# meg89/bevfusion_multimodal_3d_object_detection

Measured on AMD Instinct MI355X. Metric: BEV frames/sec (6-cam+LiDAR, 128x128 BEV), higher is better.
Workload: dtype fp32; 1 GPU; camera+LiDAR, 6x900x1600 images + 35k-point sweep, BEV 128x128; batch_per_gpu=8, parallelism=replicas x1, conv_kernels=wino, weights=random-init (synthetic, seeded), launch=eager, mode=inference forward -> 5 head tensors

## Files before the change

### bevfusion_multimodal_3d_object_detection_amd/_lib.py

```python
from __future__ import annotations

import ctypes as C
import os
from typing import Optional, Sequence

import torch

_HERE = os.path.dirname(os.path.abspath(__file__))
LIB_PATH = os.path.join(_HERE, "csrc", "libbevf_hip.so")


class BevfError(RuntimeError):
    pass


class ConvDesc(C.Structure):
    _fields_ = [("x", C.c_void_p), ("w", C.c_void_p), ("scale", C.c_void_p), ("shift", C.c_void_p),
                ("res", C.c_void_p), ("y", C.c_void_p), ("colmax", C.c_void_p)] + \
               [(n, C.c_int32) for n in ("N", "H", "W", "Cin", "x_cs", "Ho", "Wo", "Cout", "y_cs", "res_cs",
                                         "KH", "KW", "stride", "pad", "relu", "rows_per_group", "tile")] + \
               [(n, C.c_void_p) for n in ("stats", "stats_pivot", "bnb_x", "bnb_y", "bnb_mean", "bnb_invstd", "bnb_gamma",
                                          "bnb_beta")]


# ... 100 lines not shown
    "bevf_pillar_moments_f32": (C.c_int, [C.POINTER(PillarGeom)] + [C.c_void_p] * 4 + [C.c_int, C.c_float, C.c_float] +
                                [C.c_void_p] * 10),
    "bevf_pillar_pfn_backward_f32": (C.c_int, [C.POINTER(PillarGeom)] + [C.c_void_p] * 10 + [C.c_int] * 2 + [C.c_void_p] * 6),
    "bevf_resize_normalize_u8": (C.c_int, [C.c_void_p] * 2 + [C.c_int] * 5 + [C.c_void_p] * 2 + [C.c_int] + [C.c_void_p] * 2 +
                                 [C.c_int] + [C.POINTER(C.c_float)] * 2 + [C.c_void_p]),
    "bevf_lidar_filter_pad_f32": (C.c_int, [C.c_void_p] * 5 + [C.c_int] * 3 + [C.POINTER(C.c_float), C.c_void_p]),
    "bevf_resample_tables_box_f64": (C.c_int, [C.c_void_p] + [C.c_int] * 7 + [C.c_void_p] * 5),
    "bevf_resize_crop_u8": (C.c_int, [C.c_void_p] * 3 + [C.c_int] * 5 + [C.c_void_p] * 2 + [C.c_int] + [C.c_void_p] * 2 + [C.c_int] +
                            [C.c_void_p]),
    "bevf_jitter_flip_normalize_u8": (C.c_int, [C.c_void_p] * 5 + [C.c_int] * 3 + [C.POINTER(C.c_float)] * 2 + [C.c_void_p]),
    "bevf_points_affine_work_floats": (C.c_size_t, [C.c_int] * 3),
    "bevf_points_affine_filter_pad_f32": (C.c_int, [C.c_void_p] * 6 + [C.c_int] * 6 + [C.POINTER(C.c_float), C.c_void_p]),
    "bevf_points_affine_f32": (C.c_int, [C.c_void_p] * 3 + [C.c_float] + [C.c_int] * 5 + [C.c_void_p]),
    "bevf_boxes_affine_f32": (C.c_int, [C.c_void_p] * 5 + [C.c_int] * 3 + [C.c_void_p]),
    "bevf_split_weights_f32x3": (C.c_int, [C.c_void_p, C.c_void_p, C.c_size_t, C.c_void_p]),
    "bevf_conv2d_nhwc_f32x3": (C.c_int, [C.POINTER(ConvDesc), C.c_void_p]),
    "bevf_conv2d_nhwc_bf16": (C.c_int, [C.POINTER(ConvDesc), C.c_void_p]),
    "bevf_conv3x3_pack_elems": (C.c_size_t, [C.c_int] * 2),
    "bevf_conv3x3_bf16_ct": (C.c_int, [C.c_int]),
    "bevf_conv3x3_pack_bf16": (C.c_int, [C.c_void_p] * 2 + [C.c_int] * 2 + [C.c_void_p]),
    "bevf_conv3x3_bf16": (C.c_int, [C.POINTER(ConvDesc), C.c_void_p]),
    "bevf_debug_conv3x3_stamps": (C.c_int, [C.c_void_p]),
    "bevf_debug_wino_stamps": (C.c_int, [C.c_void_p]),
    "bevf_stem_pack_bf16": (C.c_int, [C.c_void_p] * 3),
    "bevf_stem_conv7x7_bf16mma": (C.c_int, [C.c_void_p] * 5 + [C.c_int] * 4 + [C.c_void_p]),
    "bevf_stem_pool_bf16mma": (C.c_int, [C.c_void_p] * 5 + [C.c_int] * 3 + [C.c_void_p]),
    "bevf_stem_conv7x7_bf16out": (C.c_int, [C.c_void_p] * 5 + [C.c_int] * 4 + [C.c_void_p]),
    "bevf_maxpool3x3s2_nhwc_bf16": (C.c_int, [C.c_void_p] * 2 + [C.c_int] * 4 + [C.c_void_p]),
    "bevf_pointwise_smallk_bf16out": (C.c_int, [C.c_void_p] * 5 + [C.c_int] * 4 + [C.c_void_p]),
    "bevf_linear_bf16w": (C.c_int, [C.c_void_p] * 4 + [C.c_int] * 7 + [C.c_void_p]),
    "bevf_cam_mean_bf16": (C.c_int, [C.c_void_p] * 2 + [C.c_int] * 4 + [C.c_void_p]),
    "bevf_bilinear_nhwc_bf16": (C.c_int, [C.c_void_p] * 2 + [C.c_int] * 8 + [C.c_void_p]),
    "bevf_broadcast_nhwc_bf16": (C.c_int, [C.c_void_p] * 2 + [C.c_int] * 4 + [C.c_void_p]),
    "bevf_expand_border_classes_bf16": (C.c_int, [C.c_void_p] * 2 + [C.c_int] * 5 + [C.c_void_p]),
    "bevf_head_tail_bf16": (C.c_int, [C.POINTER(HeadDesc), C.c_void_p]),
    "bevf_conv_pixtab_bytes": (C.c_size_t, [C.c_int] * 7),
    "bevf_conv_pixtab": (C.c_int, [C.c_void_p] + [C.c_int] * 8 + [C.c_void_p]),
    "bevf_conv2d_wgrad_f32": (C.c_int, [C.POINTER(WgradDesc), C.c_void_p]),
    "bevf_wino_wgrad_workspace_floats": (C.c_size_t, [C.c_int] * 5),
    "bevf_wino_wgrad_table_bytes": (C.c_size_t, [C.c_int] * 3),
    "bevf_wino_wgrad_table": (C.c_int, [C.c_void_p] + [C.c_int] * 5 + [C.c_void_p]),
    "bevf_conv3x3_wgrad_wino_f32": (C.c_int, [C.POINTER(WgradDesc), C.c_void_p, C.c_int, C.c_void_p]),
    "bevf_zero_stuff_nhwc_f32": (C.c_int, [C.c_void_p] * 2 + [C.c_int] * 7 + [C.c_void_p]),
    "bevf_stem_wgrad_f32": (C.c_int, [C.c_void_p] * 3 + [C.c_int] * 3 + [C.c_void_p]),
    "bevf_interleave2x2_nhwc_f32": (C.c_int, [C.c_void_p] * 4 + [C.c_int] * 4 + [C.c_void_p]),
    "bevf_bn_work_floats": (C.c_size_t, [C.c_int]),
# ... 1143 lines not shown
```

### bevfusion_multimodal_3d_object_detection_amd/csrc/conv_wino.hip

```cpp
#include "wino_common.h"

namespace {

struct WinoArgs {
  const float* x;
  const float* u;
  const float* scale;
  const float* shift;
  const float* res;
  float* y;
  float* stats;
  const float* pivot;
  const float *bnb_x, *bnb_y, *bnb_mean, *bnb_invstd, *bnb_gamma, *bnb_beta;
  int N, H, W, Cin, x_cs, Cout, y_cs, res_cs;
  int TBY, TBX, nct;
  int HS, SB;
  unsigned div_mul;
  unsigned long long* stamps;
};

constexpr int kWinoStamps = 6;

constexpr int PITCH = 36;
constexpr int PDMA = 12;
constexpr int PATCH_FLOATS = 4 * PDMA * 64 * 4;
constexpr int BG_FLOATS = 16 * 4 * 16 * 8;
constexpr int LDS_BYTES = (2 * PATCH_FLOATS + 2 * BG_FLOATS) * 4;

template <bool RES, bool RELU, bool STATS = false, int BNB = 0, int GEO = 0, bool DIAG = false>
__global__ __launch_bounds__(256, 1) void wino_f32(const WinoArgs p) {
  auto stamp_at = [&](int i, unsigned long long tm) {
    if constexpr (DIAG) {
      if (threadIdx.x == 0) p.stamps[(size_t)((blockIdx.z * gridDim.y + blockIdx.y) * gridDim.x + blockIdx.x) * kWinoStamps + i] = tm;
    }
  };
  auto stamp = [&](int i) {
    if constexpr (DIAG) stamp_at(i, __builtin_amdgcn_s_memtime());
  };
  stamp(0);
  constexpr int BHP = GEO ? 32 : 16, BWP = GEO ? 8 : 16;
  constexpr int PWP = BWP + 2, PIXG = (BHP + 2) * PWP;
  constexpr int PSLOTSG = PIXG * 9;
  static_assert(PSLOTSG <= 4 * PDMA * 64, "patch does not fit the DMA image");
  extern __shared__ __attribute__((aligned(16))) float lds[];
  float* const patch = lds;
  float* const bbuf = lds + 2 * PATCH_FLOATS;
  const int tid = threadIdx.x, lane = tid & 63;
  const int wave = __builtin_amdgcn_readfirstlane(tid >> 6);
  const int G = p.Cin >> 3;
  const int NCH = p.Cin >> 5;
  const __amdgpu_buffer_rsrc_t rsx = buf_rsrc(p.x);
  auto block_rows = [&](int sp, int& n0, int& r0, int& n, int& rb, int& hw) {
    if (p.HS) {
      const int s0 = BHP * sp - 1 + p.HS, q0 = (int)__umulhi((unsigned)s0, p.div_mul);
      n0 = q0 - 1;
      r0 = s0 - q0 * p.HS;
      hw = p.HS;
      const bool top = r0 + 1 == p.HS;
      n = top ? q0 : n0;
      rb = top ? 0 : r0 + 1;
    } else {
      n0 = p.div_mul ? (int)__umulhi((unsigned)sp, p.div_mul) : sp;
      rb = BHP * (sp - n0 * p.TBY);
      r0 = rb - 1;
      hw = 0x7fffffff;
      n = n0;
    }
  };
  auto wrap_row = [](int& row, int hw) {
    const bool wr = row >= hw;
    row -= wr ? hw : 0;
    return wr;
  };
  auto pixel_off = [&](unsigned pix, int n0, int r0, int hw, int ix0, bool& ok) {
    const unsigned py = __umul24(pix, GEO ? 6554u : 3641u) >> 16, px = pix - __umul24(py, (unsigned)PWP);
    int iy = r0 + (int)py;
    const int ix = ix0 + (int)px;
    const bool wr = wrap_row(iy, hw);
    ok = (unsigned)iy < (unsigned)p.H && (unsigned)ix < (unsigned)p.W && (unsigned)(n0 + (wr ? 1 : 0)) < (unsigned)p.N;
    const unsigned row = (unsigned)(n0 * p.H) + (wr ? (unsigned)p.H : 0u) + (unsigned)iy;
    return __umul24(__umul24(row, (unsigned)p.W) + (unsigned)ix, (unsigned)(p.x_cs * 4));
  };
  auto patch_dma_from = [&](__amdgpu_buffer_rsrc_t rs, unsigned voff, unsigned soff, int buf, int j) {
    __builtin_amdgcn_raw_ptr_buffer_load_lds(rs, (__attribute__((address_space(3))) void*)(patch + buf * PATCH_FLOATS + (4 * j + wave) * 256),
                                             16, voff, soff, 0, 0);
  };
  auto patch_dma = [&](unsigned voff, unsigned soff, int buf, int j) { patch_dma_from(rsx, voff, soff, buf, j); };
  auto make_pv = [&](unsigned (&pv)[PDMA], int& n, int& rb, int& hw, int& bx, int& ct) {
    bx = blockIdx.x;
    ct = blockIdx.z;
    int n0, r0;
    block_rows(blockIdx.y, n0, r0, n, rb, hw);
    const int ix0 = BWP * bx - 1;
#pragma unroll
    for (int j = 0; j < PDMA; ++j) {
      const unsigned sl = (unsigned)((4 * j + wave) * 64 + lane);
      const unsigned pix = __umul24(sl, 7282u) >> 16, piece = sl - 9u * pix;
      bool pok;
      const unsigned off = pixel_off(pix, n0, r0, hw, ix0, pok);
      const bool in_patch = (4 * j + 3) * 64 + 63 < PSLOTSG || sl < (unsigned)PSLOTSG;
      pv[j] = (in_patch && piece < 8u && pok) ? off + 16u * piece : kOob;
      patch_dma(pv[j], 0, 0, j);
      __builtin_amdgcn_sched_barrier(0);
    }
  };
  const __amdgpu_buffer_rsrc_t rsr_pf = buf_rsrc(RES ? p.res : p.x);
  bool pf_res = false;

  const __amdgpu_buffer_rsrc_t rsu = buf_rsrc(p.u);
  const unsigned u_lane = (unsigned)((wave * 8 * 256 + lane * 4) * 4);
  auto dma_piece = [&](unsigned img, int buf, int i) {
    __builtin_amdgcn_raw_ptr_buffer_load_lds(rsu, (__attribute__((address_space(3))) void*)(bbuf + buf * BG_FLOATS + wave * 8 * 256 + i * 256),
                                             16, u_lane, img + i * 1024, 0, 0);
  };

  const int t = lane & 15, kq = lane >> 4;
  const int ty = GEO ? 4 * wave + (t >> 2) : 2 * wave + (t >> 3), tx = GEO ? (t & 3) : (t & 7);
  const int a_lane = ((2 * ty) * PWP + 2 * tx) * PITCH + 2 * kq;
  const int b_lane = kq * 64 + t * 4;

  f32x4 acc[16][4];
  f32x2 vv[2][16], dn[16];
  auto load_patch = [&](const float* pa, int q, int c) {
    dn[4 * q + c] = *reinterpret_cast<const f32x2*>(pa + (q * PWP + c) * PITCH);
    dn[4 * q + c + 1] = *reinterpret_cast<const f32x2*>(pa + (q * PWP + c + 1) * PITCH);
  };
  auto transform_into = [&](f32x2 (&v)[16]) {
#pragma unroll
    for (int c = 0; c < 4; ++c) {
      const f32x2 t0 = dn[0 + c] - dn[8 + c], t1 = dn[4 + c] + dn[8 + c], t2 = dn[8 + c] - dn[4 + c], t3 = dn[4 + c] - dn[12 + c];
      dn[0 + c] = t0; dn[4 + c] = t1; dn[8 + c] = t2; dn[12 + c] = t3;
    }
#pragma unroll
    for (int r = 0; r < 4; ++r) {
      v[4 * r + 0] = dn[4 * r + 0] - dn[4 * r + 2];
      v[4 * r + 1] = dn[4 * r + 1] + dn[4 * r + 2];
      v[4 * r + 2] = dn[4 * r + 2] - dn[4 * r + 1];
      v[4 * r + 3] = dn[4 * r + 1] - dn[4 * r + 3];
    }
  };

  unsigned pv[PDMA], pvl[PDMA];
  int n, rb, hw, bx, ct;
  {
    const int ct0 = blockIdx.z;
#pragma unroll
    for (int i = 0; i < 8; ++i) dma_piece((unsigned)(ct0 * G) * (BG_FLOATS * 4), 0, i);
  }
  make_pv(pv, n, rb, hw, bx, ct);
  unsigned long long t_issued = 0;
  if constexpr (DIAG) t_issued = __builtin_amdgcn_s_memtime();
#pragma unroll
  for (int j = 0; j < 4; ++j) patch_dma(NCH > 1 ? pv[j] : kOob, 128, 1, j);
  asm volatile("s_waitcnt vmcnt(4) lgkmcnt(0)\n\ts_barrier" ::: "memory");
#pragma unroll
  for (int q = 0; q < 4; ++q) {
    load_patch(patch + a_lane, q, 0);
    load_patch(patch + a_lane, q, 2);
  }
  transform_into(vv[0]);
  int pbuf = 0;
  stamp_at(1, t_issued);
  stamp(2);

  auto group = [&](auto glc, auto firstc, const unsigned psoff, const unsigned bimg, const bool bnext) {
    constexpr int gl = decltype(glc)::value;
    constexpr bool kFirst = decltype(firstc)::value;
    const int abuf = gl == 3 ? pbuf ^ 1 : pbuf;
    constexpr int agl = (gl + 1) & 3;
    const float* pb = bbuf + (gl & 1) * BG_FLOATS + b_lane;
    const float* pa = patch + abuf * PATCH_FLOATS + a_lane + agl * 8;
    f32x4 b0[2], b1[2];
    b0[0] = *reinterpret_cast<const f32x4*>(pb);
    b0[1] = *reinterpret_cast<const f32x4*>(pb + 256);
#pragma unroll
    for (int f = 0; f < 16; ++f) {
      f32x4 (&bc)[2] = (f & 1) ? b1 : b0;
      f32x4 (&bn)[2] = (f & 1) ? b0 : b1;
      const f32x2 a = vv[gl & 1][f];
#pragma unroll
      for (int k = 0; k < 8; ++k) {
        const int j = k >> 2, nb = k & 3;
        if (kFirst && j == 0) MFMA0(acc[f][nb], a[j], bc[nb >> 1][(nb & 1) * 2 + j]);
        else MFMA(acc[f][nb], a[j], bc[nb >> 1][(nb & 1) * 2 + j]);
        if (k == 0 && f < 15) bn[0] = *reinterpret_cast<const f32x4*>(pb + ((f + 1) * 2) * 256);
        if (k == 1 && f < 15) bn[1] = *reinterpret_cast<const f32x4*>(pb + ((f + 1) * 2 + 1) * 256);
        if (f < 4) {
          if (k == 2) load_patch(pa, f, 0);
          if (k == 3) load_patch(pa, f, 2);
        }
        if (f == 5 && k == 2) transform_into(vv[(gl + 1) & 1]);
        if (f == 0 && bnext) dma_piece(bimg, (gl + 1) & 1, k);
        if (f == 1 && k >= 4 && gl != 2) {
          constexpr int part = gl == 3 ? 0 : gl + 1;
          if (RES && gl == 0 && pf_res) patch_dma_from(rsr_pf, pvl[part * 4 + (k - 4)], psoff, pbuf ^ 1, part * 4 + (k - 4));
          else patch_dma(pvl[part * 4 + (k - 4)], psoff, gl == 3 ? pbuf : pbuf ^ 1, part * 4 + (k - 4));
        }
        __builtin_amdgcn_sched_barrier(0);
      }
    }
    if constexpr (gl == 3) asm volatile("s_nop 15\n\ts_nop 15\n\ts_waitcnt vmcnt(4) lgkmcnt(0)\n\ts_barrier" ::: "memory");
    else asm volatile("s_waitcnt vmcnt(%0) lgkmcnt(0)\n\ts_barrier" ::"n"(gl == 2 ? 0 : 4) : "memory");
  };

  {
    using T = std::true_type;
    using F = std::false_type;
#pragma unroll
    for (int j = 0; j < PDMA; ++j) pvl[j] = pv[j];
    for (int chunk = 0; chunk < NCH; ++chunk) {
      const bool lastc = chunk + 1 == NCH;
      const unsigned ug = (unsigned)(ct * G + chunk * 4) * (BG_FLOATS * 4), gb = BG_FLOATS * 4;
      const unsigned soff = (unsigned)((chunk + 1) * 128);
      if (lastc) {
#pragma unroll
        for (int j = 4; j < PDMA; ++j) pvl[j] = kOob;
        if constexpr (RES) {
          pf_res = true;
#pragma unroll
          for (int s2 = 0; s2 < 2; ++s2) {
            const int line = s2 * 64 + lane, pw = line >> 1;
            const int prow = GEO ? (pw >> 3) : (pw >> 4), pcol = GEO ? (pw & 7) : (pw & 15);
            int ry = rb + (GEO ? 8 : 4) * wave + prow;
            const bool wr = wrap_row(ry, hw);
            const int rn = n + (wr ? 1 : 0), rx = BWP * bx + pcol;
            const bool ok = rn < p.N && ry < p.H && rx < p.W && ct * 64 + (line & 1) * 32 < p.Cout;
            pvl[4 + s2] = ok ? (unsigned)((((rn * p.H + ry) * p.W + rx) * p.res_cs + ct * 64 + (line & 1) * 32) * 4) - soff : kOob;
          }
        }
      }
      if (chunk + 2 >= NCH) {
#pragma unroll
        for (int j = 0; j < 4; ++j) pvl[j] = kOob;
      }
      if (chunk == 0) group(ic<0>{}, T{}, soff, ug + 1 * gb, true); else group(ic<0>{}, F{}, soff, ug + 1 * gb, true);
      group(ic<1>{}, F{}, soff, ug + 2 * gb, true);
      group(ic<2>{}, F{}, soff, ug + 3 * gb, true);
      group(ic<3>{}, F{}, soff + 128, ug + 4 * gb, !lastc);
      pbuf ^= 1;
    }

    asm volatile("s_waitcnt vmcnt(0)");
    stamp(3);
    if constexpr (STATS || BNB != 0) __syncthreads();
    {
      int oy = rb + (GEO ? 8 * wave + 2 * kq : 4 * wave + 2 * (kq >> 1));
      const int ox = GEO ? 8 * bx : 16 * bx + 8 * (kq & 1);
      const bool wr = wrap_row(oy, hw);
      const int nl = n + (wr ? 1 : 0);
      const bool rok[2] = {nl < p.N && oy < p.H, nl < p.N && oy + 1 < p.H};
      const bool interior = BWP * bx + BWP <= p.W && ct * 64 + 64 <= p.Cout;
      const __amdgpu_buffer_rsrc_t rsy = buf_rsrc(p.y);
      const __amdgpu_buffer_rsrc_t rsr = buf_rsrc(p.res);
      const unsigned y_lane = (unsigned)((((nl * p.H + oy) * p.W + ox) * p.y_cs + ct * 64 + t) * 4);
      const unsigned r_lane = (unsigned)((((nl * p.H + oy) * p.W + ox) * p.res_cs + ct * 64 + t) * 4);
      const unsigned yb[2] = {rok[0] ? y_lane : kOob, rok[1] ? y_lane + (unsigned)(p.W * p.y_cs * 4) : kOob};
      const unsigned rbs[2] = {rok[0] ? r_lane : kOob, rok[1] ? r_lane + (unsigned)(p.W * p.res_cs * 4) : kOob};
      auto emit = [&](auto interiorc) {
        constexpr bool kInt = decltype(interiorc)::value;
        float sc[4], sh[4];
        bool cok[4];
#pragma unroll
        for (int nb = 0; nb < 4; ++nb) {
          const int co = ct * 64 + nb * 16 + t;
          cok[nb] = kInt || co < p.Cout;
// ... 15 lines not shown
        auto fetch = [&](int nb, int set) {
#pragma unroll
          for (int q = 0; q < 16; ++q) {
            const unsigned vy = vo(nb, q, yb);
            lx[set][q] = __builtin_bit_cast(float, __builtin_amdgcn_raw_buffer_load_b32(rbx, vy, soff_of(nb, q, p.y_cs), 0));
            if constexpr (BNB == 2)
              ly[set][q] = __builtin_bit_cast(float, __builtin_amdgcn_raw_buffer_load_b32(rby, vy, soff_of(nb, q, p.y_cs), 0));
            if constexpr (RES)
              rv[set][q] = __builtin_bit_cast(float, __builtin_amdgcn_raw_buffer_load_b32(
                               rsr, vo(nb, q, rbs), soff_of(nb, q, p.res_cs), 0));
          }
        };
        auto res_fetch = [&](int nb, int set) {
#pragma unroll
          for (int q = 0; q < 16; ++q)
            rv[set][q] = __builtin_bit_cast(float, __builtin_amdgcn_raw_buffer_load_b32(rsr, vo(nb, q, rbs), soff_of(nb, q, p.res_cs), 0));
        };
        if constexpr (BNB != 0) {
          fetch(0, 0);
        } else if constexpr (RES) {
          res_fetch(0, 0);
          res_fetch(1, 1);
        }
#pragma unroll
        for (int nb = 0; nb < 4; ++nb) {
          __builtin_amdgcn_sched_barrier(0);
          if constexpr (BNB != 0) {
            if (nb < 3) fetch(nb + 1, (nb + 1) & 1);
          }
          const int set = nb & 1;
          float st1 = 0.f, st2 = 0.f;
          const int cch = ct * 64 + nb * 16 + t;
          const float pvt = (STATS && p.pivot && cok[nb]) ? p.pivot[cch] : 0.f;
          float mu = 0.f, is = 1.f, fa = 1.f, fb = 0.f;
          if constexpr (BNB != 0) {
            if (cok[nb]) {
              mu = p.bnb_mean[cch];
              is = p.bnb_invstd[cch];
              fa = (p.bnb_gamma ? p.bnb_gamma[cch] : 1.f) * is;
              fb = (p.bnb_beta ? p.bnb_beta[cch] : 0.f) - mu * fa;
            }
          }
          f32x2 sr[2][4][2];
#pragma unroll
          for (int nu = 0; nu < 4; ++nu)
#pragma unroll
            for (int hh = 0; hh < 2; ++hh) {
              const f32x2 m0 = {acc[0 + nu][nb][2 * hh], acc[0 + nu][nb][2 * hh + 1]}, m1 = {acc[4 + nu][nb][2 * hh], acc[4 + nu][nb][2 * hh + 1]};
              const f32x2 m2 = {acc[8 + nu][nb][2 * hh], acc[8 + nu][nb][2 * hh + 1]}, m3 = {acc[12 + nu][nb][2 * hh], acc[12 + nu][nb][2 * hh + 1]};
              sr[0][nu][hh] = m0 + m1 + m2;
              sr[1][nu][hh] = pk_sub<false>(pk_sub<false>(m1, m2), m3);
            }
#pragma unroll
          for (int i = 0; i < 2; ++i) {
            f32x2 yh[2][2];
#pragma unroll
            for (int hh = 0; hh < 2; ++hh) {
              yh[0][hh] = sr[i][0][hh] + sr[i][1][hh] + sr[i][2][hh];
              yh[1][hh] = pk_sub<false>(pk_sub<false>(sr[i][1][hh], sr[i][2][hh]), sr[i][3][hh]);
            }
            const f32x2 sc2 = {sc[nb], sc[nb]}, sh2 = {sh[nb], sh[nb]};
            f32x2 of[2][2];
#pragma unroll
            for (int j = 0; j < 2; ++j)
#pragma unroll
              for (int hh = 0; hh < 2; ++hh) of[j][hh] = __builtin_elementwise_fma(yh[j][hh], sc2, sh2);
#pragma unroll
            for (int j = 0; j < 2; ++j)
#pragma unroll
              for (int r = 0; r < 4; ++r) {
                const int q = r * 4 + i * 2 + j;
                float o = of[j][r >> 1][r & 1];
                if constexpr (RES) o += rv[set][q];
                if constexpr (RELU) o = fmaxf(o, 0.f);
                if constexpr (BNB != 0) {
                  const float tv = BNB == 2 ? ly[set][q] : fmaf(lx[set][q], fa, fb);
                  o = tv > 0.f ? o : 0.f;
                  if (live(nb, q)) {
                    st1 += o;
                    st2 = fmaf(o, (lx[set][q] - mu) * is, st2);
                  }
                }
                __builtin_amdgcn_raw_buffer_store_b32(__builtin_bit_cast(unsigned, o), rsy, vo(nb, q, yb), soff_of(nb, q, p.y_cs), 0);
                if constexpr (STATS) {
                  const float dv = live(nb, q) ? o - pvt : 0.f;
                  st1 += dv;
                  st2 = fmaf(dv, dv, st2);
                }
              }
          }
          if constexpr (RES && BNB == 0) {
            if (nb < 2) res_fetch(nb + 2, set);
          }
          if constexpr (STATS || BNB != 0) {
            st1 += __shfl_xor(st1, 16); st2 += __shfl_xor(st2, 16);
            st1 += __shfl_xor(st1, 32); st2 += __shfl_xor(st2, 32);
            if (kq == 0) {
              lds[(wave * 64 + nb * 16 + t) * 2] = st1;
              lds[(wave * 64 + nb * 16 + t) * 2 + 1] = st2;
            }
          }
        }
      };
      if (interior) emit(std::true_type{}); else emit(std::false_type{});
      if constexpr (DIAG) {
        stamp(4);
        asm volatile("s_waitcnt vmcnt(0)" ::: "memory");
        stamp(5);
      }
      if constexpr (STATS || BNB != 0) {
        __syncthreads();
        if (tid < 64 && ct * 64 + tid < p.Cout) {
          float a1 = 0.f, a2 = 0.f;
#pragma unroll
          for (int w = 0; w < 4; ++w) { a1 += lds[(w * 64 + tid) * 2]; a2 += lds[(w * 64 + tid) * 2 + 1]; }
          float* dst = p.stats + ((size_t)(blockIdx.y * p.TBX + blockIdx.x) * p.Cout + ct * 64 + tid) * 2;
          dst[0] = a1;
          dst[1] = a2;
        }
      }
    }
  }
}


__global__ __launch_bounds__(256) void wino_filter_transform(const float* __restrict__ w, float* __restrict__ u, int Cout,
                                                             int Cin, int nct) {
  const long long idx = blockIdx.x * 256ll + threadIdx.x;
  const long long total = (long long)nct * 64 * Cin;
  if (idx >= total) return;
  const int ci = (int)(idx % Cin), co = (int)(idx / Cin);
  double g[3][3];
#pragma unroll
  for (int i = 0; i < 3; ++i)
#pragma unroll
    for (int j = 0; j < 3; ++j) g[i][j] = co < Cout ? (double)w[(((size_t)co * 3 + i) * 3 + j) * Cin + ci] : 0.0;
  const double Gm[4][3] = {{1, 0, 0}, {.5, .5, .5}, {.5, -.5, .5}, {0, 0, 1}};
  double tmp[4][3], U[4][4];
#pragma unroll
  for (int i = 0; i < 4; ++i)
#pragma unroll
    for (int j = 0; j < 3; ++j) tmp[i][j] = Gm[i][0] * g[0][j] + Gm[i][1] * g[1][j] + Gm[i][2] * g[2][j];
#pragma unroll
  for (int i = 0; i < 4; ++i)
#pragma unroll
    for (int j = 0; j < 4; ++j) U[i][j] = tmp[i][0] * Gm[j][0] + tmp[i][1] * Gm[j][1] + tmp[i][2] * Gm[j][2];
  const int G = Cin >> 3, ct = co >> 6, nb = (co & 63) >> 4, nn = co & 15, g8 = ci >> 3, q = ci & 7;
#pragma unroll
  for (int f = 0; f < 16; ++f)
    u[((((size_t)ct * G + g8) * 16 + f) * 2 + (nb >> 1)) * 256 + ((q >> 1) * 16 + nn) * 4 + (nb & 1) * 2 + (q & 1)] =
        (float)U[f >> 2][f & 3];
}

}

static unsigned long long* g_wino_stamps = nullptr;
extern "C" int bevf_debug_wino_stamps(void* buf) {
  g_wino_stamps = static_cast<unsigned long long*>(buf);
  return BEVF_OK;
}

extern "C" int bevf_wino_stat_rows(int N, int H, int W) { return N * ((H + 15) / 16) * ((W + 15) / 16); }

extern "C" size_t bevf_wino_filter_floats(int Cout, int Cin) {
  return (size_t)((Cout + 63) / 64) * 64 * 16 * (size_t)Cin;
}

extern "C" int bevf_wino_filter_transform_f32(const float* w_ohwi, float* u, int Cout, int Cin, void* stream) {
  BEVF_REQUIRE(w_ohwi && u, "wino_filter_transform: null pointer");
  BEVF_REQUIRE(Cout > 0 && Cin > 0 && Cin % 32 == 0, "wino_filter_transform: Cin=%d must be a positive multiple of 32", Cin);
  const int nct = (Cout + 63) / 64;
  const long long total = (long long)nct * 64 * Cin;
  return bevf_launch("bevf_wino_filter_transform_f32", wino_filter_transform, dim3((unsigned)((total + 255) / 256)), dim3(256), 0,
                     static_cast<hipStream_t>(stream), w_ohwi, u, Cout, Cin, nct);
}

// ... 31 lines not shown
    long long best = (long long)a.SB * a.TBX;
    for (int cand = 1; cand < 4; ++cand) {
      const int bh = (cand & 1) ? 32 : 16, bw = (cand & 1) ? 8 : 16, tbx = (d->W + bw - 1) / bw;
      if ((cand & 2) && (hs <= bh || (long long)d->N * hs >= (1ll << 30))) continue;
      const long long sb = (cand & 2) ? ((long long)d->N * hs - (hs - d->H) + bh - 1) / bh : (long long)d->N * ((d->H + bh - 1) / bh);
      const bool forced = d->tile == cand + 1;
      if (d->tile != 0 && !forced) continue;
      if (forced || sb * tbx < best) {
        best = sb * tbx;
        geo1 = cand & 1;
        a.TBY = (d->H + bh - 1) / bh; a.TBX = tbx; a.SB = (int)sb; a.HS = (cand & 2) ? hs : 0;
      }
    }
  }
  const long long ntiles = (long long)a.SB * a.TBX * a.nct;
  BEVF_REQUIRE(ntiles < (1ll << 31) && a.SB < 65536 && a.nct < 65536, "conv_wino: too many tiles");
  {
    const unsigned long long dv = a.HS ? (unsigned long long)a.HS : (unsigned long long)a.TBY;
    const unsigned long long top = a.HS ? (unsigned long long)a.SB * (geo1 ? 32 : 16) + dv : (unsigned long long)a.SB;
    BEVF_REQUIRE((top + dv) * dv < (1ull << 32), "conv_wino: map too tall for the row arithmetic");
    a.div_mul = (unsigned)(((1ull << 32) + dv - 1) / dv);
  }
  hipStream_t st = static_cast<hipStream_t>(stream);
  const dim3 grid((unsigned)a.TBX, (unsigned)a.SB, (unsigned)a.nct), block(256);
  auto go = [&](auto kern) { return bevf_launch("bevf_conv3x3_wino_f32", kern, grid, block, LDS_BYTES, st, a); };
  if (d->bnb_x)
    return bevf_dispatch_bool(d->res != nullptr, [&](auto R) {
      constexpr bool res = decltype(R)::value;
      return d->bnb_y ? go(&wino_f32<res, false, false, 2>) : go(&wino_f32<res, false, false, 1>);
    });
  if (d->stats) return go(&wino_f32<false, false, true>);
  const bool diag = g_wino_stamps && d->relu;
  if (diag) a.stamps = g_wino_stamps;
  return bevf_dispatch_bool(d->res != nullptr, [&](auto R) {
    return bevf_dispatch_bool(geo1, [&](auto G) {
      constexpr bool res = decltype(R)::value;
      constexpr int geo = decltype(G)::value;
      if (diag) return go(&wino_f32<res, true, false, 0, geo, true>);
      return d->relu ? go(&wino_f32<res, true, false, 0, geo>) : go(&wino_f32<res, false, false, 0, geo>);
    });
  });
}
```

### bevfusion_multimodal_3d_object_detection_amd/csrc/wino_common.h

```cpp
#pragma once
#include "conv_common.h"

namespace {

typedef float f32x2 __attribute__((ext_vector_type(2)));

#define MFMA(acc_, a_, b_) asm volatile("v_mfma_f32_16x16x4_f32 %0, %1, %2, %0" : "+a"(acc_) : "v"(a_), "v"(b_))
#define MFMA0(acc_, a_, b_) asm volatile("v_mfma_f32_16x16x4_f32 %0, %1, %2, 0" : "=a"(acc_) : "v"(a_), "v"(b_))

template <bool PINNED>
__device__ __forceinline__ f32x2 pk_sub(f32x2 a, f32x2 b) {
  f32x2 d;
  if constexpr (PINNED) asm volatile("v_pk_add_f32 %0, %1, %2 neg_lo:[0,1] neg_hi:[0,1]" : "=v"(d) : "v"(a), "v"(b));
  else asm("v_pk_add_f32 %0, %1, %2 neg_lo:[0,1] neg_hi:[0,1]" : "=v"(d) : "v"(a), "v"(b));
  return d;
}

}
```

### include/bevf.h

```cpp
#ifndef BEVF_H
#define BEVF_H

#include <stddef.h>
#include <stdint.h>

#ifdef __cplusplus
extern "C" {
#endif

typedef enum {
  BEVF_OK = 0,
  BEVF_ERR_ARG = -1,
  BEVF_ERR_LAUNCH = -2,
  BEVF_ERR_UNSUPPORTED = -3
} bevf_status;

int bevf_version(void);
const char* bevf_last_error(void);

typedef struct {
  const float* x;
  const float* w;
  const float* scale;
  const float* shift;
// ... 213 lines not shown
                          int C, void* stream);

int bevf_frustum_table_sort_wave_rows(void);
size_t bevf_frustum_table_work_elems(int B, int ncam, int bev_h, int bev_w, int D, int Hc, int Wc);
int bevf_frustum_table_build_f64(const double* calib, int B, int ncam, float x0, float y0, float vx, float vy, int bev_h,
                                 int bev_w, float z0, float z1, int D, double depth_min, double depth_max, int img_h,
                                 int img_w, int Hc, int Wc, int32_t* cell_of, int32_t* row_ptr, int32_t* col2, void* work,
                                 void* stream);
int bevf_frustum_pool_f32(const int32_t* row_ptr, size_t rp_stride, const int32_t* col2, size_t e_stride, int nrows, int D,
                          const float* x, size_t x_bs, int x_cs, const float* pd, size_t pd_bs, float* y, size_t y_bs,
                          int y_cs, int B, int C, void* stream);
int bevf_frustum_pool_bwd_f32(const int32_t* cell_of, size_t c_stride, int npix, int D, const float* x, size_t x_bs, int x_cs,
                              const float* pd, size_t pd_bs, const float* dy, size_t dy_bs, int dy_cs, float* dx,
                              size_t dx_bs, int dx_cs, float* dpd, size_t dpd_bs, int B, int C, void* stream);

int bevf_conv2d_nhwc_bf16(const bevf_conv_desc* d, void* stream);

size_t bevf_conv3x3_pack_elems(int Cout, int Cin);
int bevf_conv3x3_bf16_ct(int Cout);
int bevf_conv3x3_pack_bf16(const void* w_ohwi, void* packed, int Cout, int Cin, void* stream);
int bevf_conv3x3_bf16(const bevf_conv_desc* d, void* stream);
int bevf_debug_conv3x3_stamps(void* buf);
int bevf_debug_wino_stamps(void* buf);

int bevf_split_weights_f32x3(const float* w, void* planes, size_t n, void* stream);
int bevf_conv2d_nhwc_f32x3(const bevf_conv_desc* d, void* stream);
int bevf_stem_conv7x7_bf16out(const float* x, const float* w, const float* scale, const float* shift, void* y, int N,
                              int H, int W, int relu, void* stream);
int bevf_stem_pack_bf16(const float* w_oihw, void* packed, void* stream);
int bevf_stem_conv7x7_bf16mma(const float* x, const void* w_packed, const float* scale, const float* shift, void* y,
                              int N, int H, int W, int relu, void* stream);
int bevf_stem_pool_bf16mma(const float* x, const void* w_packed, const float* scale, const float* shift, void* y, int N,
                           int H, int W, void* stream);
int bevf_maxpool3x3s2_nhwc_bf16(const void* x, void* y, int N, int H, int W, int C, void* stream);
int bevf_pointwise_smallk_bf16out(const float* x, const float* w, const float* scale, const float* shift, void* y,
                                  int M, int K, int Cout, int relu, void* stream);
int bevf_linear_bf16w(const float* x, const void* w, const float* bias, void* y, int y_bf16, int B, int K, int O,
                      int relu, int perm_inner, int perm_outer, void* stream);
int bevf_cam_mean_bf16(const void* x, void* y, int B, int ncam, int P, int C, void* stream);
int bevf_bilinear_nhwc_bf16(const void* x, void* y, int B, int Hi, int Wi, int C, int x_cs, int Ho, int Wo, int y_cs,
                            void* stream);
int bevf_broadcast_nhwc_bf16(const float* v, void* y, int B, int P, int C, int y_cs, void* stream);
int bevf_expand_border_classes_bf16(const void* small, void* y, int B, int Sh, int Sw, int C, int y_cs, void* stream);
int bevf_head_tail_bf16(const bevf_head_desc* d, void* stream);


// ... 110 lines not shown
```

Baseline: 292.1 frames/s.

## Make Winograd conv persistent with run-on tiles prefetching the next tile's patch

Adds a persistent-kernel mode to the Winograd fp32 conv: the grid becomes one workgroup per CU, and each workgroup loops over tiles. The next tile's input patch and weight DMA are issued during the last chunks of the current tile, so each new tile's load overlaps the previous tile's tail and epilogue. Accumulators are pinned to named AGPRs via inline asm so the run-on loop keeps them in fixed registers. The mode is enabled only when the tile count divides evenly across CUs or is large, and only for plain epilogues. It adds risk in the hand-managed vmcnt waits and register pressure, and the residual prefetch becomes a dummy load.

```diff
diff --git a/bevfusion_multimodal_3d_object_detection_amd/_lib.py b/bevfusion_multimodal_3d_object_detection_amd/_lib.py
--- a/bevfusion_multimodal_3d_object_detection_amd/_lib.py
+++ b/bevfusion_multimodal_3d_object_detection_amd/_lib.py
@@ -146,6 +146,7 @@
     "bevf_conv3x3_bf16": (C.c_int, [C.POINTER(ConvDesc), C.c_void_p]),
     "bevf_debug_conv3x3_stamps": (C.c_int, [C.c_void_p]),
     "bevf_debug_wino_stamps": (C.c_int, [C.c_void_p]),
+    "bevf_debug_wino_workgroups": (C.c_int, [C.c_int]),
     "bevf_stem_pack_bf16": (C.c_int, [C.c_void_p] * 3),
     "bevf_stem_conv7x7_bf16mma": (C.c_int, [C.c_void_p] * 5 + [C.c_int] * 4 + [C.c_void_p]),
     "bevf_stem_pool_bf16mma": (C.c_int, [C.c_void_p] * 5 + [C.c_int] * 3 + [C.c_void_p]),
diff --git a/bevfusion_multimodal_3d_object_detection_amd/csrc/conv_wino.hip b/bevfusion_multimodal_3d_object_detection_amd/csrc/conv_wino.hip
--- a/bevfusion_multimodal_3d_object_detection_amd/csrc/conv_wino.hip
+++ b/bevfusion_multimodal_3d_object_detection_amd/csrc/conv_wino.hip
@@ -1,4 +1,7 @@
 #include "wino_common.h"
+
+#include <map>
+#include <mutex>
 
 namespace {
 
@@ -16,6 +19,8 @@
   int TBY, TBX, nct;
   int HS, SB;
   unsigned div_mul;
+  int ntiles, nsp;
+  unsigned nsp_mul, tbx_mul;
   unsigned long long* stamps;
 };
 
@@ -27,8 +32,9 @@
 constexpr int BG_FLOATS = 16 * 4 * 16 * 8;
 constexpr int LDS_BYTES = (2 * PATCH_FLOATS + 2 * BG_FLOATS) * 4;
 
-template <bool RES, bool RELU, bool STATS = false, int BNB = 0, int GEO = 0, bool DIAG = false>
+template <bool RES, bool RELU, bool STATS = false, int BNB = 0, int GEO = 0, bool DIAG = false, bool RUNON = false>
 __global__ __launch_bounds__(256, 1) void wino_f32(const WinoArgs p) {
+  static_assert(!RUNON || (!STATS && BNB == 0 && !DIAG), "the run-on tile loop has no barrier after a tile: plain epilogues only");
   auto stamp_at = [&](int i, unsigned long long tm) {
     if constexpr (DIAG) {
       if (threadIdx.x == 0) p.stamps[(size_t)((blockIdx.z * gridDim.y + blockIdx.y) * gridDim.x + blockIdx.x) * kWinoStamps + i] = tm;
@@ -37,7 +43,8 @@
   auto stamp = [&](int i) {
     if constexpr (DIAG) stamp_at(i, __builtin_amdgcn_s_memtime());
   };
-  stamp(0);
+  unsigned long long t_start = 0;
+  if constexpr (DIAG) t_start = __builtin_amdgcn_s_memtime();
   constexpr int BHP = GEO ? 32 : 16, BWP = GEO ? 8 : 16;
   constexpr int PWP = BWP + 2, PIXG = (BHP + 2) * PWP;
   constexpr int PSLOTSG = PIXG * 9;
@@ -49,6 +56,12 @@
   const int wave = __builtin_amdgcn_readfirstlane(tid >> 6);
   const int G = p.Cin >> 3;
   const int NCH = p.Cin >> 5;
+  auto tile_of = [&](int lt, int& bx, int& sp, int& ct) {
+    ct = p.nsp_mul ? (int)__umulhi((unsigned)lt, p.nsp_mul) : lt;
+    const int rem = lt - ct * p.nsp;
+    sp = p.tbx_mul ? (int)__umulhi((unsigned)rem, p.tbx_mul) : rem;
+    bx = rem - sp * p.TBX;
+  };
   const __amdgpu_buffer_rsrc_t rsx = buf_rsrc(p.x);
   auto block_rows = [&](int sp, int& n0, int& r0, int& n, int& rb, int& hw) {
     if (p.HS) {
@@ -86,11 +99,9 @@
                                              16, voff, soff, 0, 0);
   };
   auto patch_dma = [&](unsigned voff, unsigned soff, int buf, int j) { patch_dma_from(rsx, voff, soff, buf, j); };
-  auto make_pv = [&](unsigned (&pv)[PDMA], int& n, int& rb, int& hw, int& bx, int& ct) {
-    bx = blockIdx.x;
-    ct = blockIdx.z;
+  auto make_pv = [&](unsigned (&pv)[PDMA], auto issuec, int bx, int sp, int& n, int& rb, int& hw) {
     int n0, r0;
-    block_rows(blockIdx.y, n0, r0, n, rb, hw);
+    block_rows(sp, n0, r0, n, rb, hw);
     const int ix0 = BWP * bx - 1;
 #pragma unroll
     for (int j = 0; j < PDMA; ++j) {
@@ -100,12 +111,25 @@
       const unsigned off = pixel_off(pix, n0, r0, hw, ix0, pok);
       const bool in_patch = (4 * j + 3) * 64 + 63 < PSLOTSG || sl < (unsigned)PSLOTSG;
       pv[j] = (in_patch && piece < 8u && pok) ? off + 16u * piece : kOob;
-      patch_dma(pv[j], 0, 0, j);
-      __builtin_amdgcn_sched_barrier(0);
+      if constexpr (decltype(issuec)::value) {
+        patch_dma(pv[j], 0, 0, j);
+        __builtin_amdgcn_sched_barrier(0);
+      }
     }
   };
   const __amdgpu_buffer_rsrc_t rsr_pf = buf_rsrc(RES ? p.res : p.x);
   bool pf_res = false;
+  unsigned pfv[2] = {kOob, kOob};
+  unsigned junk[2] = {0u, 0u};
+  auto res_line = [&](int s2, int n, int rb, int hw, int bx, int ct) {
+    const int line = s2 * 64 + lane, pw = line >> 1;
+    const int prow = GEO ? (pw >> 3) : (pw >> 4), pcol = GEO ? (pw & 7) : (pw & 15);
+    int ry = rb + (GEO ? 8 : 4) * wave + prow;
+    const bool wr = wrap_row(ry, hw);
+    const int rn = n + (wr ? 1 : 0), rx = BWP * bx + pcol;
+    const bool ok = rn < p.N && ry < p.H && rx < p.W && ct * 64 + (line & 1) * 32 < p.Cout;
+    return ok ? (unsigned)((((rn * p.H + ry) * p.W + rx) * p.res_cs + ct * 64 + (line & 1) * 32) * 4) : kOob;
+  };
 
   const __amdgpu_buffer_rsrc_t rsu = buf_rsrc(p.u);
   const unsigned u_lane = (unsigned)((wave * 8 * 256 + lane * 4) * 4);
@@ -119,7 +143,6 @@
   const int a_lane = ((2 * ty) * PWP + 2 * tx) * PITCH + 2 * kq;
   const int b_lane = kq * 64 + t * 4;
 
-  f32x4 acc[16][4];
   f32x2 vv[2][16], dn[16];
   auto load_patch = [&](const float* pa, int q, int c) {
     dn[4 * q + c] = *reinterpret_cast<const f32x2*>(pa + (q * PWP + c) * PITCH);
@@ -140,18 +163,37 @@
     }
   };
 
-  unsigned pv[PDMA], pvl[PDMA];
-  int n, rb, hw, bx, ct;
+  unsigned pv[PDMA], pvn[PDMA], pvl[PDMA];
+  int n, rb, hw, bx, ct, sp;
+  int nn = 0, rbn = 0, hwn = 0, bxn = 0, ctn = 0;
+  int lt = blockIdx.x;
+  bool has_next = false;
+  if constexpr (RUNON) {
+    tile_of(lt, bx, sp, ct);
+  } else {
+    bx = blockIdx.x; sp = blockIdx.y; ct = blockIdx.z;
+  }
   {
-    const int ct0 = blockIdx.z;
-#pragma unroll
-    for (int i = 0; i < 8; ++i) dma_piece((unsigned)(ct0 * G) * (BG_FLOATS * 4), 0, i);
-  }
-  make_pv(pv, n, rb, hw, bx, ct);
+#pragma unroll
+    for (int i = 0; i < 8; ++i) dma_piece((unsigned)(ct * G) * (BG_FLOATS * 4), 0, i);
+  }
+  make_pv(pv, std::true_type{}, bx, sp, n, rb, hw);
+  auto make_next = [&]() {
+    has_next = lt + (int)gridDim.x < p.ntiles;
+    if (has_next) {
+      int spn;
+      tile_of(lt + (int)gridDim.x, bxn, spn, ctn);
+      make_pv(pvn, std::false_type{}, bxn, spn, nn, rbn, hwn);
+    } else {
+#pragma unroll
+      for (int j = 0; j < PDMA; ++j) pvn[j] = kOob;
+    }
+  };
   unsigned long long t_issued = 0;
   if constexpr (DIAG) t_issued = __builtin_amdgcn_s_memtime();
 #pragma unroll
   for (int j = 0; j < 4; ++j) patch_dma(NCH > 1 ? pv[j] : kOob, 128, 1, j);
+  if constexpr (RUNON) make_next();
   asm volatile("s_waitcnt vmcnt(4) lgkmcnt(0)\n\ts_barrier" ::: "memory");
 #pragma unroll
   for (int q = 0; q < 4; ++q) {
@@ -160,6 +202,7 @@
   }
   transform_into(vv[0]);
   int pbuf = 0;
+  stamp_at(0, t_start);
   stamp_at(1, t_issued);
   stamp(2);
 
@@ -173,74 +216,96 @@
     f32x4 b0[2], b1[2];
     b0[0] = *reinterpret_cast<const f32x4*>(pb);
     b0[1] = *reinterpret_cast<const f32x4*>(pb + 256);
-#pragma unroll
-    for (int f = 0; f < 16; ++f) {
+    static_for<16>([&](auto fc) {
+      constexpr int f = decltype(fc)::value;
       f32x4 (&bc)[2] = (f & 1) ? b1 : b0;
       f32x4 (&bn)[2] = (f & 1) ? b0 : b1;
       const f32x2 a = vv[gl & 1][f];
-#pragma unroll
-      for (int k = 0; k < 8; ++k) {
-        const int j = k >> 2, nb = k & 3;
-        if (kFirst && j == 0) MFMA0(acc[f][nb], a[j], bc[nb >> 1][(nb & 1) * 2 + j]);
-        else MFMA(acc[f][nb], a[j], bc[nb >> 1][(nb & 1) * 2 + j]);
-        if (k == 0 && f < 15) bn[0] = *reinterpret_cast<const f32x4*>(pb + ((f + 1) * 2) * 256);
-        if (k == 1 && f < 15) bn[1] = *reinterpret_cast<const f32x4*>(pb + ((f + 1) * 2 + 1) * 256);
-        if (f < 4) {
-          if (k == 2) load_patch(pa, f, 0);
-          if (k == 3) load_patch(pa, f, 2);
-        }
-        if (f == 5 && k == 2) transform_into(vv[(gl + 1) & 1]);
-        if (f == 0 && bnext) dma_piece(bimg, (gl + 1) & 1, k);
-        if (f == 1 && k >= 4 && gl != 2) {
+      static_for<8>([&](auto kc) {
+        constexpr int k = decltype(kc)::value, j = k >> 2, nb = k & 3;
+        mfma_named<16 * f + 4 * nb, kFirst && j == 0>(a[j], bc[nb >> 1][(nb & 1) * 2 + j]);
+        if constexpr (k == 0 && f < 15) bn[0] = *reinterpret_cast<const f32x4*>(pb + ((f + 1) * 2) * 256);
+        if constexpr (k == 1 && f < 15) bn[1] = *reinterpret_cast<const f32x4*>(pb + ((f + 1) * 2 + 1) * 256);
+        if constexpr (f < 4) {
+          if constexpr (k == 2) load_patch(pa, f, 0);
+          if constexpr (k == 3) load_patch(pa, f, 2);
+        }
+        if constexpr (f == 5 && k == 2) transform_into(vv[(gl + 1) & 1]);
+        if constexpr (f == 0) {
+          if (bnext) dma_piece(bimg, (gl + 1) & 1, k);
+        }
+        if constexpr (f == 1 && k >= 4 && gl != 2) {
           constexpr int part = gl == 3 ? 0 : gl + 1;
-          if (RES && gl == 0 && pf_res) patch_dma_from(rsr_pf, pvl[part * 4 + (k - 4)], psoff, pbuf ^ 1, part * 4 + (k - 4));
+          if (RES && !RUNON && gl == 0 && pf_res) patch_dma_from(rsr_pf, pvl[part * 4 + (k - 4)], psoff, pbuf ^ 1, part * 4 + (k - 4));
           else patch_dma(pvl[part * 4 + (k - 4)], psoff, gl == 3 ? pbuf : pbuf ^ 1, part * 4 + (k - 4));
         }
+        if constexpr (RES && RUNON && gl == 0 && f == 2 && k < 2)
+          junk[k] = __builtin_amdgcn_raw_buffer_load_b32(rsr_pf, pfv[k], 0, 0);
         __builtin_amdgcn_sched_barrier(0);
-      }
-    }
+      });
+    });
     if constexpr (gl == 3) asm volatile("s_nop 15\n\ts_nop 15\n\ts_waitcnt vmcnt(4) lgkmcnt(0)\n\ts_barrier" ::: "memory");
-    else asm volatile("s_waitcnt vmcnt(%0) lgkmcnt(0)\n\ts_barrier" ::"n"(gl == 2 ? 0 : 4) : "memory");
-  };
-
-  {
+    else asm volatile("s_waitcnt vmcnt(%0) lgkmcnt(0)\n\ts_barrier" ::"n"(gl == 2 ? 0 : (RES && RUNON && gl == 0) ? 6 : 4) : "memory");
+    if constexpr (RES && RUNON && gl == 2) asm volatile("" ::"v"(junk[0]), "v"(junk[1]));
+  };
+
+  for (;;) {
     using T = std::true_type;
     using F = std::false_type;
-#pragma unroll
-    for (int j = 0; j < PDMA; ++j) pvl[j] = pv[j];
+    if constexpr (!RUNON) {
+#pragma unroll
+      for (int j = 0; j < PDMA; ++j) pvl[j] = pv[j];
+    }
     for (int chunk = 0; chunk < NCH; ++chunk) {
       const bool lastc = chunk + 1 == NCH;
       const unsigned ug = (unsigned)(ct * G + chunk * 4) * (BG_FLOATS * 4), gb = BG_FLOATS * 4;
-      const unsigned soff = (unsigned)((chunk + 1) * 128);
-      if (lastc) {
-#pragma unroll
-        for (int j = 4; j < PDMA; ++j) pvl[j] = kOob;
+      unsigned soff = (unsigned)((chunk + 1) * 128), soff3 = soff + 128;
+      unsigned bimg3 = ug + 4 * gb;
+      bool bnext3 = !lastc;
+      if constexpr (RUNON) {
+        const bool nextc = chunk + 2 >= NCH;
+#pragma unroll
+        for (int j = 0; j < 4; ++j) pvl[j] = nextc ? pvn[j] : pv[j];
+#pragma unroll
+        for (int j = 4; j < PDMA; ++j) pvl[j] = lastc ? pvn[j] : pv[j];
+        soff = lastc ? 0u : soff;
+        soff3 = nextc ? (unsigned)((chunk + 2 - NCH) * 128) : soff3;
+        bimg3 = lastc ? (unsigned)(ctn * G) * (BG_FLOATS * 4) : bimg3;
+        bnext3 = !lastc || has_next;
         if constexpr (RES) {
-          pf_res = true;
-#pragma unroll
-          for (int s2 = 0; s2 < 2; ++s2) {
-            const int line = s2 * 64 + lane, pw = line >> 1;
-            const int prow = GEO ? (pw >> 3) : (pw >> 4), pcol = GEO ? (pw & 7) : (pw & 15);
-            int ry = rb + (GEO ? 8 : 4) * wave + prow;
-            const bool wr = wrap_row(ry, hw);
-            const int rn = n + (wr ? 1 : 0), rx = BWP * bx + pcol;
-            const bool ok = rn < p.N && ry < p.H && rx < p.W && ct * 64 + (line & 1) * 32 < p.Cout;
-            pvl[4 + s2] = ok ? (unsigned)((((rn * p.H + ry) * p.W + rx) * p.res_cs + ct * 64 + (line & 1) * 32) * 4) - soff : kOob;
-          }
-        }
-      }
-      if (chunk + 2 >= NCH) {
-#pragma unroll
-        for (int j = 0; j < 4; ++j) pvl[j] = kOob;
+#pragma unroll
+          for (int s2 = 0; s2 < 2; ++s2) pfv[s2] = kOob;
+          if (lastc) {
+#pragma unroll
+            for (int s2 = 0; s2 < 2; ++s2) pfv[s2] = res_line(s2, n, rb, hw, bx, ct);
+          }
+        }
+      } else {
+        if (lastc) {
+#pragma unroll
+          for (int j = 4; j < PDMA; ++j) pvl[j] = kOob;
+          if constexpr (RES) {
+            pf_res = true;
+#pragma unroll
+            for (int s2 = 0; s2 < 2; ++s2) {
+              const unsigned ro = res_line(s2, n, rb, hw, bx, ct);
+              pvl[4 + s2] = ro != kOob ? ro - soff : kOob;
+            }
+          }
+        }
+        if (chunk + 2 >= NCH) {
+#pragma unroll
+          for (int j = 0; j < 4; ++j) pvl[j] = kOob;
+        }
       }
       if (chunk == 0) group(ic<0>{}, T{}, soff, ug + 1 * gb, true); else group(ic<0>{}, F{}, soff, ug + 1 * gb, true);
       group(ic<1>{}, F{}, soff, ug + 2 * gb, true);
       group(ic<2>{}, F{}, soff, ug + 3 * gb, true);
-      group(ic<3>{}, F{}, soff + 128, ug + 4 * gb, !lastc);
+      group(ic<3>{}, F{}, soff3, bimg3, bnext3);
       pbuf ^= 1;
     }
 
-    asm volatile("s_waitcnt vmcnt(0)");
+    if (!RUNON || !has_next) asm volatile("s_waitcnt vmcnt(0)");
     stamp(3);
     if constexpr (STATS || BNB != 0) __syncthreads();
     {
@@ -302,8 +367,8 @@
           res_fetch(0, 0);
           res_fetch(1, 1);
         }
-#pragma unroll
-        for (int nb = 0; nb < 4; ++nb) {
+        static_for<4>([&](auto nbc) {
+          constexpr int nb = decltype(nbc)::value;
           __builtin_amdgcn_sched_barrier(0);
           if constexpr (BNB != 0) {
             if (nb < 3) fetch(nb + 1, (nb + 1) & 1);
@@ -322,15 +387,14 @@
             }
           }
           f32x2 sr[2][4][2];
-#pragma unroll
-          for (int nu = 0; nu < 4; ++nu)
-#pragma unroll
-            for (int hh = 0; hh < 2; ++hh) {
-              const f32x2 m0 = {acc[0 + nu][nb][2 * hh], acc[0 + nu][nb][2 * hh + 1]}, m1 = {acc[4 + nu][nb][2 * hh], acc[4 + nu][nb][2 * hh + 1]};
-              const f32x2 m2 = {acc[8 + nu][nb][2 * hh], acc[8 + nu][nb][2 * hh + 1]}, m3 = {acc[12 + nu][nb][2 * hh], acc[12 + nu][nb][2 * hh + 1]};
-              sr[0][nu][hh] = m0 + m1 + m2;
-              sr[1][nu][hh] = pk_sub<false>(pk_sub<false>(m1, m2), m3);
-            }
+          static_for<8>([&](auto nhc) {
+            constexpr int nu = decltype(nhc)::value >> 1, hh = decltype(nhc)::value & 1;
+            constexpr int r0 = 16 * nu + 4 * nb + 2 * hh;
+            const f32x2 m0 = {acc_named<r0>(), acc_named<r0 + 1>()}, m1 = {acc_named<r0 + 64>(), acc_named<r0 + 65>()};
+            const f32x2 m2 = {acc_named<r0 + 128>(), acc_named<r0 + 129>()}, m3 = {acc_named<r0 + 192>(), acc_named<r0 + 193>()};
+            sr[0][nu][hh] = m0 + m1 + m2;
+            sr[1][nu][hh] = pk_sub<false>(pk_sub<false>(m1, m2), m3);
+          });
 #pragma unroll
           for (int i = 0; i < 2; ++i) {
             f32x2 yh[2][2];
@@ -354,7 +418,7 @@
                 if constexpr (RES) o += rv[set][q];
                 if constexpr (RELU) o = fmaxf(o, 0.f);
                 if constexpr (BNB != 0) {
-                  const float tv = BNB == 2 ? ly[set][q] : fmaf(lx[set][q], fa, fb);
+                  const float tv = BNB == 2 ? ly[BNB == 2 ? set : 0][q] : fmaf(lx[set][q], fa, fb);
                   o = tv > 0.f ? o : 0.f;
                   if (live(nb, q)) {
                     st1 += o;
@@ -380,7 +444,7 @@
               lds[(wave * 64 + nb * 16 + t) * 2 + 1] = st2;
             }
           }
-        }
+        });
       };
       if (interior) emit(std::true_type{}); else emit(std::false_type{});
       if constexpr (DIAG) {
@@ -400,6 +464,16 @@
         }
       }
     }
+    if constexpr (!RUNON) {
+      break;
+    } else {
+      if (!has_next) break;
+      lt += (int)gridDim.x;
+      n = nn; rb = rbn; hw = hwn; bx = bxn; ct = ctn;
+#pragma unroll
+      for (int j = 0; j < PDMA; ++j) pv[j] = pvn[j];
+      make_next();
+    }
   }
 }
 
@@ -432,6 +506,38 @@
         (float)U[f >> 2][f & 3];
 }
 
+}
+
+static int g_wino_workgroups = 0;
+extern "C" int bevf_debug_wino_workgroups(int n) {
+  BEVF_REQUIRE(n >= 0, "bevf_debug_wino_workgroups: n=%d < 0", n);
+  g_wino_workgroups = n;
+  return BEVF_OK;
+}
+
+static int wino_cu_count(int* out) {
+  static std::mutex mu;
+  static std::map<int, int> known;
+  int dev = 0;
+  hipError_t e = hipGetDevice(&dev);
+  if (e == hipSuccess) {
+    std::lock_guard<std::mutex> lock(mu);
+    const auto it = known.find(dev);
+    if (it != known.end()) {
+      *out = it->second;
+      return BEVF_OK;
+    }
+    int cus = 0;
+    e = hipDeviceGetAttribute(&cus, hipDeviceAttributeMultiprocessorCount, dev);
+    if (e == hipSuccess && cus > 0) {
+      known[dev] = cus;
+      *out = cus;
+      return BEVF_OK;
+    }
+  }
+  (void)hipGetLastError();
+  bevf_set_error("conv_wino: cannot read the device's compute-unit count: %s", hipGetErrorString(e));
+  return BEVF_ERR_LAUNCH;
 }
 
 static unsigned long long* g_wino_stamps = nullptr;
@@ -509,7 +615,27 @@
     a.div_mul = (unsigned)(((1ull << 32) + dv - 1) / dv);
   }
   hipStream_t st = static_cast<hipStream_t>(stream);
-  const dim3 grid((unsigned)a.TBX, (unsigned)a.SB, (unsigned)a.nct), block(256);
+  dim3 grid((unsigned)a.TBX, (unsigned)a.SB, (unsigned)a.nct);
+  const dim3 block(256);
+  const bool diag = g_wino_stamps && d->relu;
+  a.ntiles = (int)ntiles; a.nsp = a.SB * a.TBX; a.nsp_mul = a.tbx_mul = 0;
+  bool runon = false;
+  if (!d->stats && !d->bnb_x && !diag && d->Cin >= 64) {
+    int wgs = g_wino_workgroups;
+    bool pays = true;
+    if (wgs == 0) {
+      const int rc = wino_cu_count(&wgs);
+      if (rc != BEVF_OK) return rc;
+      pays = ntiles % wgs == 0 || ntiles >= 8ll * wgs;
+    }
+    const unsigned long long nsp = (unsigned long long)a.nsp, tbx = (unsigned long long)a.TBX;
+    if (pays && wgs < ntiles && ((unsigned long long)ntiles + nsp) * nsp < (1ull << 32) && (nsp + tbx) * tbx < (1ull << 32)) {
+      runon = true;
+      if (nsp > 1) a.nsp_mul = (unsigned)(((1ull << 32) + nsp - 1) / nsp);
+      if (tbx > 1) a.tbx_mul = (unsigned)(((1ull << 32) + tbx - 1) / tbx);
+      grid = dim3((unsigned)wgs);
+    }
+  }
   auto go = [&](auto kern) { return bevf_launch("bevf_conv3x3_wino_f32", kern, grid, block, LDS_BYTES, st, a); };
   if (d->bnb_x)
     return bevf_dispatch_bool(d->res != nullptr, [&](auto R) {
@@ -517,14 +643,16 @@
       return d->bnb_y ? go(&wino_f32<res, false, false, 2>) : go(&wino_f32<res, false, false, 1>);
     });
   if (d->stats) return go(&wino_f32<false, false, true>);
-  const bool diag = g_wino_stamps && d->relu;
   if (diag) a.stamps = g_wino_stamps;
   return bevf_dispatch_bool(d->res != nullptr, [&](auto R) {
     return bevf_dispatch_bool(geo1, [&](auto G) {
       constexpr bool res = decltype(R)::value;
       constexpr int geo = decltype(G)::value;
       if (diag) return go(&wino_f32<res, true, false, 0, geo, true>);
-      return d->relu ? go(&wino_f32<res, true, false, 0, geo>) : go(&wino_f32<res, false, false, 0, geo>);
+      return bevf_dispatch_bool(runon, [&](auto O) {
+        constexpr bool ro = decltype(O)::value;
+        return d->relu ? go(&wino_f32<res, true, false, 0, geo, false, ro>) : go(&wino_f32<res, false, false, 0, geo, false, ro>);
+      });
     });
   });
 }
diff --git a/bevfusion_multimodal_3d_object_detection_amd/csrc/wino_common.h b/bevfusion_multimodal_3d_object_detection_amd/csrc/wino_common.h
--- a/bevfusion_multimodal_3d_object_detection_amd/csrc/wino_common.h
+++ b/bevfusion_multimodal_3d_object_detection_amd/csrc/wino_common.h
@@ -8,6 +8,38 @@
 #define MFMA(acc_, a_, b_) asm volatile("v_mfma_f32_16x16x4_f32 %0, %1, %2, %0" : "+a"(acc_) : "v"(a_), "v"(b_))
 #define MFMA0(acc_, a_, b_) asm volatile("v_mfma_f32_16x16x4_f32 %0, %1, %2, 0" : "=a"(acc_) : "v"(a_), "v"(b_))
 
+#define WINO_MFMA_AT_(r0, r1, r2, r3)                                                                                              \
+  else if constexpr (R == r0) {                                                                                                    \
+    if constexpr (ZERO) asm volatile("v_mfma_f32_16x16x4_f32 a[%0:%1], %2, %3, 0" ::"n"(r0), "n"(r3), "v"(a), "v"(b) : "a" #r0, "a" #r1, "a" #r2, "a" #r3); \
+    else asm volatile("v_mfma_f32_16x16x4_f32 a[%0:%1], %2, %3, a[%0:%1]" ::"n"(r0), "n"(r3), "v"(a), "v"(b) : "a" #r0, "a" #r1, "a" #r2, "a" #r3); \
+  }
+#define WINO_MFMA_ALL_ \
+  WINO_MFMA_AT_(0, 1, 2, 3) WINO_MFMA_AT_(4, 5, 6, 7) WINO_MFMA_AT_(8, 9, 10, 11) WINO_MFMA_AT_(12, 13, 14, 15) WINO_MFMA_AT_(16, 17, 18, 19) WINO_MFMA_AT_(20, 21, 22, 23) \
+  WINO_MFMA_AT_(24, 25, 26, 27) WINO_MFMA_AT_(28, 29, 30, 31) WINO_MFMA_AT_(32, 33, 34, 35) WINO_MFMA_AT_(36, 37, 38, 39) WINO_MFMA_AT_(40, 41, 42, 43) WINO_MFMA_AT_(44, 45, 46, 47) \
+  WINO_MFMA_AT_(48, 49, 50, 51) WINO_MFMA_AT_(52, 53, 54, 55) WINO_MFMA_AT_(56, 57, 58, 59) WINO_MFMA_AT_(60, 61, 62, 63) WINO_MFMA_AT_(64, 65, 66, 67) WINO_MFMA_AT_(68, 69, 70, 71) \
+  WINO_MFMA_AT_(72, 73, 74, 75) WINO_MFMA_AT_(76, 77, 78, 79) WINO_MFMA_AT_(80, 81, 82, 83) WINO_MFMA_AT_(84, 85, 86, 87) WINO_MFMA_AT_(88, 89, 90, 91) WINO_MFMA_AT_(92, 93, 94, 95) \
+  WINO_MFMA_AT_(96, 97, 98, 99) WINO_MFMA_AT_(100, 101, 102, 103) WINO_MFMA_AT_(104, 105, 106, 107) WINO_MFMA_AT_(108, 109, 110, 111) WINO_MFMA_AT_(112, 113, 114, 115) WINO_MFMA_AT_(116, 117, 118, 119) \
+  WINO_MFMA_AT_(120, 121, 122, 123) WINO_MFMA_AT_(124, 125, 126, 127) WINO_MFMA_AT_(128, 129, 130, 131) WINO_MFMA_AT_(132, 133, 134, 135) WINO_MFMA_AT_(136, 137, 138, 139) WINO_MFMA_AT_(140, 141, 142, 143) \
+  WINO_MFMA_AT_(144, 145, 146, 147) WINO_MFMA_AT_(148, 149, 150, 151) WINO_MFMA_AT_(152, 153, 154, 155) WINO_MFMA_AT_(156, 157, 158, 159) WINO_MFMA_AT_(160, 161, 162, 163) WINO_MFMA_AT_(164, 165, 166, 167) \
+  WINO_MFMA_AT_(168, 169, 170, 171) WINO_MFMA_AT_(172, 173, 174, 175) WINO_MFMA_AT_(176, 177, 178, 179) WINO_MFMA_AT_(180, 181, 182, 183) WINO_MFMA_AT_(184, 185, 186, 187) WINO_MFMA_AT_(188, 189, 190, 191) \
+  WINO_MFMA_AT_(192, 193, 194, 195) WINO_MFMA_AT_(196, 197, 198, 199) WINO_MFMA_AT_(200, 201, 202, 203) WINO_MFMA_AT_(204, 205, 206, 207) WINO_MFMA_AT_(208, 209, 210, 211) WINO_MFMA_AT_(212, 213, 214, 215) \
+  WINO_MFMA_AT_(216, 217, 218, 219) WINO_MFMA_AT_(220, 221, 222, 223) WINO_MFMA_AT_(224, 225, 226, 227) WINO_MFMA_AT_(228, 229, 230, 231) WINO_MFMA_AT_(232, 233, 234, 235) WINO_MFMA_AT_(236, 237, 238, 239) \
+  WINO_MFMA_AT_(240, 241, 242, 243) WINO_MFMA_AT_(244, 245, 246, 247) WINO_MFMA_AT_(248, 249, 250, 251) WINO_MFMA_AT_(252, 253, 254, 255)
+template <int R, bool ZERO>
+__device__ __forceinline__ void mfma_named(float a, float b) {
+  static_assert(R >= 0 && R % 4 == 0 && R + 3 < 256, "accumulator register range");
+  if constexpr (false) {
+  }
+  WINO_MFMA_ALL_
+}
+template <int R>
+__device__ __forceinline__ float acc_named() {
+  static_assert(R >= 0 && R < 256, "accumulator register");
+  float v;
+  asm volatile("v_accvgpr_read_b32 %0, a[%1]" : "=v"(v) : "n"(R));
+  return v;
+}
+
 template <bool PINNED>
 __device__ __forceinline__ f32x2 pk_sub(f32x2 a, f32x2 b) {
   f32x2 d;
diff --git a/include/bevf.h b/include/bevf.h
--- a/include/bevf.h
+++ b/include/bevf.h
@@ -259,6 +259,7 @@
 int bevf_conv3x3_bf16(const bevf_conv_desc* d, void* stream);
 int bevf_debug_conv3x3_stamps(void* buf);
 int bevf_debug_wino_stamps(void* buf);
+int bevf_debug_wino_workgroups(int n);
 
 int bevf_split_weights_f32x3(const float* w, void* planes, size_t n, void* stream);
 int bevf_conv2d_nhwc_f32x3(const bevf_conv_desc* d, void* stream);
```

Measured after the change: 297.4 frames/s, median of 6. +1.8%, better.
